# mohwald/gandtr

Hardware: AMD Instinct MI355X
Metric: images/sec generator@256^2 + descriptors/sec GeM-R101@1024^2, 1/2/4/8 MI355X (higher is better)
Workload: dtype f16c; 1 GPU; cyclegan ResnetGenerator 9-block (InstanceNorm) forward, synthetic 3x256x256, random-init weights; batch_per_gpu=64, global_batch=64, parallelism=dp1

## Files before the change

gandtr_amd/csrc/aux_kernels.hip:

```cpp
#include "gdt_common.h"
#include "aux_kernels.h"

namespace {

__device__ __forceinline__ void load8(const f16* p, float (&v)[8]) {
    const f16x8 t = *(const f16x8*)p;
#pragma unroll
    for (int e = 0; e < 8; ++e) v[e] = (float)t[e];
}
__device__ __forceinline__ void load8(const float* p, float (&v)[8]) {
    const float4 a = *(const float4*)p, b = *(const float4*)(p + 4);
    v[0] = a.x; v[1] = a.y; v[2] = a.z; v[3] = a.w; v[4] = b.x; v[5] = b.y; v[6] = b.z; v[7] = b.w;
}
__device__ __forceinline__ void store8(f16* p, const float (&v)[8]) {
    f16x8 t;
#pragma unroll
    for (int e = 0; e < 8; ++e) t[e] = (f16)v[e];
    *(f16x8*)p = t;
}
__device__ __forceinline__ void store8(float* p, const float (&v)[8]) {
    *(float4*)p = make_float4(v[0], v[1], v[2], v[3]);
    *(float4*)(p + 4) = make_float4(v[4], v[5], v[6], v[7]);
}

// ... 99 lines not shown
    var = var < 0.0 ? 0.0 : var;
    mean_rstd[(long)i * 2 + 0] = (float)m;
    mean_rstd[(long)i * 2 + 1] = (float)(1.0 / sqrt(var + (double)eps));
}

__global__ __launch_bounds__(1024) void in_finalize_tiles_kernel(const float* __restrict__ partial, float* __restrict__ mean_rstd,
                                                                 int tpi, int nphase, int N, int C, int HW, float eps) {
    constexpr int RL = 16;
    __shared__ double red[2][RL][64];
    const int n = blockIdx.y, c = blockIdx.x * 64 + (threadIdx.x & 63), lanegrp = threadIdx.x >> 6;
    double s = 0.0, q = 0.0;
    if (c < C) {
        const int nrec = nphase * tpi;
        auto rec = [&](int r, float& a, float& b) {
            if (r < nrec) {
                const int ph = r / tpi, t = r - ph * tpi;
                const long tile = (long)ph * N * tpi + (long)n * tpi + t;
                a = partial[(tile * 2 + 0) * C + c]; b = partial[(tile * 2 + 1) * C + c];
            } else { a = 0.f; b = 0.f; }
        };
        for (int r = lanegrp; r < nrec; r += 4 * RL) {
            float a0, b0, a1, b1, a2, b2, a3, b3;
            rec(r, a0, b0); rec(r + RL, a1, b1); rec(r + 2 * RL, a2, b2); rec(r + 3 * RL, a3, b3);
            s += (double)a0; q += (double)b0; s += (double)a1; q += (double)b1;
            s += (double)a2; q += (double)b2; s += (double)a3; q += (double)b3;
        }
    }
    red[0][lanegrp][threadIdx.x & 63] = s; red[1][lanegrp][threadIdx.x & 63] = q;
    __syncthreads();
    if (threadIdx.x < 64 && c < C) {
        s = 0.0; q = 0.0;
#pragma unroll
        for (int l = 0; l < RL; ++l) { s += red[0][l][threadIdx.x]; q += red[1][l][threadIdx.x]; }
        const double m = s / HW;
        double var = q / HW - m * m;
        var = var < 0.0 ? 0.0 : var;
        mean_rstd[((long)n * C + c) * 2 + 0] = (float)m;
        mean_rstd[((long)n * C + c) * 2 + 1] = (float)(1.0 / sqrt(var + (double)eps));
    }
}

template <typename T>
__global__ __launch_bounds__(256) void in_apply_kernel(const T* __restrict__ x, const float* __restrict__ mean_rstd,
                                                       const T* __restrict__ res, T* __restrict__ y,
                                                       long HW, int C, int relu, long total8) {
    const int c8n = C >> 3;
    for (long i = (long)blockIdx.x * 256 + threadIdx.x; i < total8; i += (long)gridDim.x * 256) {
        const int c8 = (int)(i % c8n);
        const long n = (i / c8n) / HW;
        const float* mr = mean_rstd + (n * C + c8 * 8) * 2;
        float v[8], r[8];
        load8(x + i * 8, v);
        if (res) load8(res + i * 8, r);
#pragma unroll
        for (int e = 0; e < 8; ++e) {
            float f = (v[e] - mr[2 * e]) * mr[2 * e + 1];
            if (relu) f = fmaxf(f, 0.f);
            if (res) f += r[e];
            v[e] = f;
        }
        store8(y + i * 8, v);
    }
}

template <typename T>
__global__ __launch_bounds__(256) void maxpool_kernel(const T* __restrict__ x, T* __restrict__ y, int N, int H, int W,
                                                      int C, int OH, int OW, int k, int s, int p) {
    const int c8n = C >> 3;
    const long total = (long)N * OH * OW * c8n;
    for (long i = (long)blockIdx.x * 256 + threadIdx.x; i < total; i += (long)gridDim.x * 256) {
        const int c8 = (int)(i % c8n);
// ... 542 lines not shown
```

gandtr_amd/csrc/conv3x3_halo_c16.hip:

```cpp
#include <cstdio>
#include <cstdlib>

#include <vector>

#include "gdt_common.h"

#ifndef GDT_C16_SCHED
#define GDT_C16_SCHED 1
#endif
#ifndef GDT_C16_RING
#define GDT_C16_RING 3
#endif
#ifndef GDT_C16_FULL_LINES
#define GDT_C16_FULL_LINES 1
#endif
#ifndef GDT_C16_BQ_SETS
#define GDT_C16_BQ_SETS 1
#endif
#ifndef GDT_C16_ABL
#define GDT_C16_ABL 0
#endif

namespace {

// ... 74 lines not shown
        int rx = ix < 0 ? -ix : (ix >= d.W ? 2 * d.W - 2 - ix : ix);
        ry = min(max(ry, 0), d.H - 1); rx = min(max(rx, 0), d.W - 1);
        const bool inb = ((unsigned)iy < (unsigned)d.H) & ((unsigned)ix < (unsigned)d.W);
        Pend p;
        p.goff = (((unsigned)((ta.n * d.H + ry) * d.W + rx) << (d.lc8 + 5)) + cbyte);
        p.ok = (h < HROWS) & (inb | refl);
        p.r0 = *(const float4*)((const char*)inf + p.goff); p.r1 = *(const float4*)((const char*)inf + p.goff + 16);
        if (RES) { p.s0 = *(const float4*)((const char*)resf + p.goff); p.s1 = *(const float4*)((const char*)resf + p.goff + 16); }
        return p;
    };
    Pend pendv[SDIST];
    auto load_piece_part = [&](const TileAt& ta, int chunk, int r, int part) {
        Pend& pend = pendv[r % SDIST];
        if (part == 0) {
            int lr = lrow;
            asm volatile("" : "+v"(lr));
            const int h = min(r * RPR + lr, HROWS_PAD - 1);
            const int hy = (h * 3641) >> 16, hx = h - hy * HW_;
            const int iy = ta.y0 - 1 + hy, ix = ta.x0 - 1 + hx;
            int ry = iy < 0 ? -iy : (iy >= d.H ? 2 * d.H - 2 - iy : iy);
            int rx = ix < 0 ? -ix : (ix >= d.W ? 2 * d.W - 2 - ix : ix);
            ry = min(max(ry, 0), d.H - 1); rx = min(max(rx, 0), d.W - 1);
            const bool inb = ((unsigned)iy < (unsigned)d.H) & ((unsigned)ix < (unsigned)d.W);
            pend.goff = (((unsigned)((ta.n * d.H + ry) * d.W + rx) << (d.lc8 + 5)) + (chunk * 8 + (lane & 7)) * 32);
            pend.ok = (h < HROWS) & (inb | refl);
            pend.r0 = *(const float4*)((const char*)inf + pend.goff);
        }
        if (part == 1) pend.r1 = *(const float4*)((const char*)inf + pend.goff + 16);
        if (RES && part == 2) pend.s0 = *(const float4*)((const char*)resf + pend.goff);
        if (RES && part == 3) pend.s1 = *(const float4*)((const char*)resf + pend.goff + 16);
    };
    float* nlds = (float*)(smem + 2 * STAGE_BYTES);
    auto stage_norm = [&](const TileAt& ta, int slot) {
        for (int i = tid; i < d.Cin / 2; i += NT) {
            const float4 v = *(const float4*)(d.in_norm + (long)ta.n * d.Cin * 2 + i * 4);
            *(float4*)(nlds + slot * 512 + i * 4) = make_float4(v.y, -v.x * v.y, v.w, -v.z * v.w);
        }
    };
    float4 nf[4];
    auto load_nf = [&](int slot, int chunk) {
        if (!NORM) return;
        const float4* np4 = (const float4*)(nlds + slot * 512 + (chunk * 8 + (lane & 7)) * 16);
#pragma unroll
        for (int k = 0; k < 4; ++k) nf[k] = np4[k];
    };
    auto store_piece = [&](int stage_off, int r, const Pend& p) {
        const int row = min(r * RPR + lrow, HROWS_PAD - 1);
        const int phy = (row * 3641) >> 16, phx = row - phy * HW_;
        float a[8] = {p.r0.x, p.r0.y, p.r0.z, p.r0.w, p.r1.x, p.r1.y, p.r1.z, p.r1.w};
        if (NORM) {
            const float lo = d.in_relu ? 0.f : -3.0e38f;
#pragma unroll
            for (int k = 0; k < 4; ++k) {
                const float4 v = nf[k];
                a[2 * k] = fmaxf(fmaf(a[2 * k], v.x, v.y), lo);
                a[2 * k + 1] = fmaxf(fmaf(a[2 * k + 1], v.z, v.w), lo);
            }
            if (RES) {
                a[0] += p.s0.x; a[1] += p.s0.y; a[2] += p.s0.z; a[3] += p.s0.w;
                a[4] += p.s1.x; a[5] += p.s1.y; a[6] += p.s1.z; a[7] += p.s1.w;
            }
        }
        if (WB) {
            *(float4*)((char*)wbf + p.goff) = make_float4(a[0], a[1], a[2], a[3]);
            *(float4*)((char*)wbf + p.goff + 16) = make_float4(a[4], a[5], a[6], a[7]);
        }
// ... 441 lines not shown
```

gandtr_amd/csrc/gdt_common.h:

```cpp
#pragma once
#include <hip/hip_runtime.h>
#include <hip/hip_fp16.h>
#include <stdint.h>
#include <mutex>
#include <string>

typedef _Float16 f16;
typedef f16 f16x8 __attribute__((ext_vector_type(8)));
typedef f16 f16x4 __attribute__((ext_vector_type(4)));
typedef f16 f16x2 __attribute__((ext_vector_type(2)));
typedef float f32x16 __attribute__((ext_vector_type(16)));
typedef float f32x4 __attribute__((ext_vector_type(4)));

void gdt_set_error(const std::string& msg);
#define GDT_OK 0
#define GDT_ERR_INVALID 1
#define GDT_ERR_HIP 2
#define GDT_ERR_WORKSPACE 3
#ifndef GDT_ERR_NOT_CONVERGED
#define GDT_ERR_NOT_CONVERGED 4
#endif

#define GDT_CHECK_HIP(expr)                                                                     \
    do {                                                                                        \
// ... 47 lines not shown
    float* stats;
    const f16* zeros;
    const float* in_norm;
    int in_relu;
    const f16* w_frag;
    const f16* in_res;
    f16* in_out;
    int N, H, W, Cin, lc8;
    int Cout, CoutPad, Kpad, nk;
    int OHg, OWg, OH, OW;
    int sy, sx, osy, ooy, osx, oox;
    int ntaps, TW, invTW, dy0, dys, dx0, dxs;
    int pad_reflect;
    int relu;
    int act;
    int M;
    int dbg;
    unsigned long long* stamp_out;
    int stats_tile_base;
    int pool2;
    const f16* w_frag2;
    const void* w_cfrag;
    const void* wmx_a; const void* wmx_b; const void* wmx_s;
    const void* w_c16;
    int pair_cout, ooy2, oox2;
    int x3_form;
    int in_f32;
    int stagger_us;
    int phase_cout;
    const f16* in2; int in2_cin, in2_h, in2_w, in2_stride;
    const f16* x_w_frag; const f16* x_bias; int x_cout;
    const f16* r_w_frag; const float* r_bias; f16* r_out;
    float group_factor;
};

constexpr int GDT_MAX_LEVELS = 4;

constexpr int GDT_C_HI_SCALE_OFF = 11;
__device__ __forceinline__ int gdt_c_pixel_exp(const float (&a)[8]) {
    const float m = fmaxf(fmaxf(fmaxf(fabsf(a[0]), fabsf(a[1])), fmaxf(fabsf(a[2]), fabsf(a[3]))),
                          fmaxf(fmaxf(fabsf(a[4]), fabsf(a[5])), fmaxf(fabsf(a[6]), fabsf(a[7]))));
    int b = __float_as_int(m);
    b = max(b, __builtin_amdgcn_mov_dpp(b, 0xB1, 0xF, 0xF, false));
    b = max(b, __builtin_amdgcn_mov_dpp(b, 0x4E, 0xF, 0xF, false));
    b = max(b, __builtin_amdgcn_mov_dpp(b, 0x141, 0xF, 0xF, false));
    return min(max((b >> 23) - 127, -14), 15);
}
__device__ __forceinline__ float gdt_exp2i(int e) { return __int_as_float((e + 127) << 23); }
struct MultiConv {
    int nlev;
    int prefix[GDT_MAX_LEVELS + 1];
    int vblocks[GDT_MAX_LEVELS];
    ConvLaunch lev[GDT_MAX_LEVELS];
};
static_assert(sizeof(MultiConv) <= 4096, "kernel arguments are limited to 4 KB");
__device__ __forceinline__ int gdt_multi_level(const int nlev, const int* prefix, const int b) {
    int l = 0;
#pragma unroll
    for (int k = 1; k < GDT_MAX_LEVELS; ++k) l += (k < nlev && b >= prefix[k]) ? 1 : 0;
    return l;
}
inline int gdt_multi_partition(int* prefix, const int* vb, int L, int slots) {
    long total = 0;
    for (int l = 0; l < L; ++l) total += vb[l];
    prefix[0] = 0;
    for (int l = 0; l < L; ++l) {
        int g = vb[l];
        if (total > slots) {
            g = (int)((long)slots * vb[l] / total) / 8 * 8;
            if (g < 8) g = 8;
            if (g > vb[l]) g = vb[l];
        }
        prefix[l + 1] = prefix[l] + g;
    }
    return prefix[L];
}

__device__ __forceinline__ bool gdt_tile_of_block(int b, int ntm, int ntn, int& tile_m, int& tile_n) {
    const int mchunk = (ntm + 7) >> 3;
    const int xcd = b & 7, j = b >> 3;
    tile_n = j % ntn;
// ... 69 lines not shown
```

gandtr_amd/csrc/net.hip:

```cpp
#include <algorithm>
#include <cmath>
#include <cstdlib>
#include <cstring>
#include <memory>
#include <vector>

#include "../../include/gandtr_hip.h"
#include "aux_kernels.h"
#include "gdt_common.h"

static thread_local std::string g_last_error;
void gdt_set_error(const std::string& msg) { g_last_error = msg; }

namespace {

constexpr size_t ALIGN = 256;
inline size_t align_up(size_t v) { return (v + ALIGN - 1) / ALIGN * ALIGN; }
inline int next_pow2(int v) { int p = 8; while (p < v) p <<= 1; return p; }
inline int ilog2(int v) { int l = 0; while ((1 << l) < v) ++l; return l; }

enum OpKind { OP_INPUT, OP_CONV, OP_INORM, OP_MAXPOOL, OP_GEM, OP_OUT_NCHW, OP_HED, OP_RCF, OP_POOL_HEAD };

struct PackedPhase {
    size_t w_off = 0;
// ... 108 lines not shown
    int last_joined = 0, last_level_launches = 0;

    size_t blob_append(const void* data, size_t bytes) {
        const size_t off = align_up(host_blob.size());
        host_blob.resize(off + bytes);
        if (data) memcpy(host_blob.data() + off, data, bytes);
        else memset(host_blob.data() + off, 0, bytes);
        return off;
    }
    int new_tensor(int C, int Creal) { tensors.push_back(Tensor{C, Creal}); return (int)tensors.size() - 1; }
};

namespace {

struct Step {
    int op; size_t aux_off[8]; bool fused_stats; int tiles_per_image;
    int norm_into;
    int norm_from;
    bool wb;
    bool ctf;
    bool aug;
    bool s2;
    bool ctp;
    int pool_into;
    bool skip;
    bool bneck;
    int bneck_ds;
    int bneck_a;
    bool xexp;
    int xchain;
    bool kcat;
    bool direct;
    int stats_sets;
};
struct Plan { std::vector<Step> steps; size_t peak = 0; };

int pool_out_dim(const Op& o, int in) {
    const int span = in + 2 * o.p - o.k + (o.ceil ? o.s - 1 : 0);
    if (span < 0) return 0;
    int out = span / o.s + 1;
    if (o.ceil && (out - 1) * o.s >= in + o.p) --out;
    return out;
}

int conv_out_dim(const Op& o, int in, int k) {
    const gdt_conv_desc& c = o.cd;
    if (c.transposed) return in * 2;
    const int span = in + 2 * c.pad - (o.dil * (k - 1) + 1);
    return span < 0 ? 0 : span / c.stride + 1;
}

void conv_geometry(const gdt_net* net, const Op& o, const PackedPhase& ph, int n, const Tensor& ti, ConvLaunch& d) {
    d.N = n; d.H = ti.H; d.W = ti.W; d.Cin = o.cin_pad; d.lc8 = ilog2(o.cin_pad / 8);
    d.Cout = o.cd.cout; d.CoutPad = o.cout_pad;
    d.OH = conv_out_dim(o, ti.H, o.cd.kh); d.OW = conv_out_dim(o, ti.W, o.cd.kw);
    d.pad_reflect = o.cd.pad_reflect; d.relu = o.cd.relu; d.act = o.cd.act;
    d.Kpad = ph.Kpad; d.nk = ph.Kpad / (net->precision ? 32 : 64);
    d.ntaps = ph.ntaps; d.TW = ph.TW; d.invTW = (65536 + ph.TW - 1) / ph.TW;
    d.dy0 = ph.dy0; d.dys = ph.dys; d.dx0 = ph.dx0; d.dxs = ph.dxs;
    if (o.cd.transposed) {
        d.OHg = ti.H; d.OWg = ti.W; d.sy = d.sx = 1; d.osy = d.osx = 2; d.ooy = ph.ooy; d.oox = ph.oox;
    } else {
        d.OHg = d.OH; d.OWg = d.OW; d.sy = d.sx = o.cd.stride; d.osy = d.osx = 1; d.ooy = d.oox = 0;
    }
    d.M = n * d.OHg * d.OWg;
}
// ... 216 lines not shown
            d.w_frag = (const f16*)net; d.out = (f16*)net;
            d.stats = conv_fuses_stats(ok, T[ok.in]) ? (float*)net : nullptr;
            ConvLaunch dn = d; dn.in_norm = (const float*)net; dn.in_res = oj.res >= 0 ? (const f16*)net : nullptr;
            const bool ok_fold = consumers[oj.out] == 1 && (gdt_conv_halo_ct_eligible(dn) || (oj.res < 0 && gdt_conv_igemm_rb_eligible(dn)));
            if (ok_fold) { plan.steps[j].norm_into = k; plan.steps[k].norm_from = j; plan.steps[j].wb = false; }
            continue;
        }
        conv_geometry(net, ok, ok.phases[0], N, T[ok.in], d);
        if (ok.rowsplit) { d.Cout = ok.rs_cout8; d.out_f32 = nullptr; }
        d.w_lo = net->precision ? (const f16*)net : nullptr;
        d.w_frag = ok.phases[0].has_frag ? (const f16*)net : nullptr;
        d.out = (ok.cd.out_f32_nchw || ok.rowsplit) ? nullptr : (f16*)net;
        d.stats = conv_fuses_stats(ok, T[ok.in]) ? (float*)net : nullptr;
        d.out_f32 = (ok.cd.out_f32_nchw && !ok.rowsplit) ? (float*)net : nullptr;
        const bool fold = net->precision ? (((x3_fold >= 2 || (!wb && oj.res < 0)) && gdt_conv_halo_x3_eligible(d)) ||
                                            (x3_fold >= 2 && !wb && oj.res < 0 && !ok.rowsplit && !ok.cd.out_f32_nchw && gdt_conv_x3_norm_eligible(d)))
                                         : (gdt_conv_halo_eligible(d) || (!wb && (gdt_conv_igemm_norm_eligible(d) || irb_norm_ok(d))));
        if (fold) { plan.steps[j].norm_into = k; plan.steps[k].norm_from = j; plan.steps[j].wb = wb; }
        static const bool plan_dbg = getenv("GDT_PLAN_DEBUG") != nullptr;
        if (plan_dbg) fprintf(stderr, "[plan] inorm %d -> conv %d: Cin %d s%d k%d rowsplit %d fold %d\n", j, k, d.Cin, ok.cd.stride, ok.cd.kh, (int)ok.rowsplit, (int)fold);
    }

    for (int i = 0; i < nops; ++i) {
        const Op& o = ops[i];
        if (o.kind != OP_CONV || plan.steps[i].ctf || o.cd.transposed || o.rowsplit || o.cd.out_f32_nchw || net->precision) continue;
        if (!conv_fuses_stats(o, T[o.in])) continue;
        ConvLaunch d{};
        conv_geometry(net, o, o.phases[0], N, T[o.in], d);
        d.w_frag = o.phases[0].has_frag ? (const f16*)net : nullptr; d.out = (f16*)net; d.stats = (float*)net;
        d.in_norm = plan.steps[i].norm_from >= 0 ? (const float*)net : nullptr;
        if (plan.steps[i].norm_from >= 0 && plan.steps[plan.steps[i].norm_from].wb) continue;
        if (!gdt_conv_stem_eligible(d) && !gdt_conv_halo_rb_eligible(d) && !gdt_conv_halo_eligible(d) && gdt_conv_igemm_rb_eligible(d))
            plan.steps[i].stats_sets = gdt_conv_igemm_rb_stats_sets(d);
    }

    for (int j = 0; j < nops; ++j) {
        const Op& oj = ops[j];
        if (oj.kind != OP_MAXPOOL || oj.k != 2 || oj.s != 2 || oj.p != 0 || net->precision || consumers[oj.in] != 1) continue;
        if (oj.ceil && ((T[oj.in].H & 1) || (T[oj.in].W & 1))) continue;
        int i = -1;
        for (int k = 0; k < j; ++k) if (ops[k].kind == OP_CONV && ops[k].out == oj.in) i = k;
        if (i < 0 || ops[i].cd.transposed || ops[i].cd.out_f32_nchw || ops[i].res >= 0 || ops[i].dil != 1) continue;
        ConvLaunch d{};
        conv_geometry(net, ops[i], ops[i].phases[0], N, T[ops[i].in], d);
        d.w_frag = ops[i].phases[0].has_frag ? (const f16*)net : nullptr; d.out = (f16*)net;
        d.in_norm = plan.steps[i].norm_from >= 0 ? (const float*)net : nullptr;
        d.stats = conv_fuses_stats(ops[i], T[ops[i].in]) ? (float*)net : nullptr;
        if (plan.steps[i].norm_from >= 0 && plan.steps[plan.steps[i].norm_from].wb) continue;
        if (gdt_conv_pool2_eligible(d)) { plan.steps[i].pool_into = j; plan.steps[j].skip = true; }
    }

    for (int i = 0; i + 2 < nops && !net->precision; ++i) {
        const Op &a = ops[i], &b = ops[i + 1], &c = ops[i + 2];
        if (a.kind != OP_CONV || b.kind != OP_CONV || c.kind != OP_CONV) continue;
        auto plain = [&](const Op& o) { return o.dil == 1 && !o.cd.transposed && !o.cd.out_f32_nchw && !o.rowsplit && o.stats_for < 0 && o.cd.stride == 1 && o.phases.size() == 1 && o.phases[0].has_frag && o.has_bias; };
        if (!plain(a) || !plain(b) || !plain(c)) continue;
        if (a.cd.kh != 1 || a.cd.kw != 1 || a.cd.pad != 0 || !a.cd.relu || a.res >= 0) continue;
        if (b.cd.kh != 3 || b.cd.kw != 3 || b.cd.pad != 1 || b.cd.pad_reflect || !b.cd.relu || b.res >= 0 || b.in != a.out) continue;
        if (c.cd.kh != 1 || c.cd.kw != 1 || c.cd.pad != 0 || !c.cd.relu || c.in != b.out || c.res != a.in) continue;
        if (consumers[a.out] != 1 || consumers[b.out] != 1) continue;
        if (plan.steps[i].norm_from >= 0 || plan.steps[i + 1].norm_from >= 0 || plan.steps[i + 2].norm_from >= 0) continue;
        if (plan.steps[i].pool_into >= 0 || plan.steps[i + 1].pool_into >= 0 || plan.steps[i + 2].pool_into >= 0) continue;
        const int C = a.cd.cin, mid = a.cd.cout;
        if (a.cin_pad != C || a.cout_pad != mid || b.cd.cin != mid || b.cd.cout != mid || b.cout_pad != mid || c.cd.cin != mid || c.cd.cout != C || c.cout_pad != C) continue;
        if (!gdt_bneck_eligible(C, C, mid, N, T[a.in].H, T[a.in].W)) continue;
        plan.steps[i].bneck = true; plan.steps[i + 1].skip = true; plan.steps[i + 2].skip = true;
// ... 134 lines not shown
                        t2.off = arena.alloc(t2.bytes);
                    }
                    break;
                }
                if (st.pool_into >= 0) {
                    Tensor& t = T[ops[st.pool_into].out];
                    t.bytes = (size_t)N * t.H * t.W * t.C * net->esize();
                    t.off = arena.alloc(t.bytes);
                } else if (o.out >= 0) alloc_out();
                if (o.rowsplit) {
                    const size_t b = (size_t)N * oh * ti.W * o.rs_cout8 * net->esize();
                    st.aux_off[1] = arena.alloc(b);
                    arena.release(st.aux_off[1], b);
                }
                if (conv_fuses_stats(o, ti)) {
                    const int hwg = o.cd.transposed ? ti.H * ti.W : oh * conv_out_dim(o, ti.W, o.cd.kw);
                    const size_t tiles = (size_t)st.stats_sets * N * (hwg / 128);
                    st.fused_stats = true; st.tiles_per_image = hwg / 128;
                    slab_bytes[i] = tiles * 2 * o.cd.cout * sizeof(float);
                    st.aux_off[0] = arena.alloc(slab_bytes[i]);
                    slab_off[i] = st.aux_off[0];
                }
                break;
            }
            case OP_INORM: {
                const Tensor& ti = T[o.in];
                const size_t mr_bytes = (size_t)N * ti.C * 2 * sizeof(float);
                if (st.norm_into < 0 || st.wb) alloc_out();
                st.aux_off[1] = arena.alloc(mr_bytes);
                if (o.stats_from >= 0 && slab_bytes[o.stats_from]) {
                    st.fused_stats = true;
                    st.tiles_per_image = plan.steps[o.stats_from].tiles_per_image;
                    st.aux_off[0] = slab_off[o.stats_from];
                    arena.release(slab_off[o.stats_from], slab_bytes[o.stats_from]);
                } else {
                    const int chunks = gdt_in_stats_chunks(ti.H * ti.W);
                    st.aux_off[0] = arena.alloc((size_t)N * chunks * 2 * ti.C * sizeof(float));
                    arena.release(st.aux_off[0], (size_t)N * chunks * 2 * ti.C * sizeof(float));
                }
                if (st.norm_into >= 0) deferred[st.norm_into].push_back({st.aux_off[1], mr_bytes});
                else arena.release(st.aux_off[1], mr_bytes);
                break;
            }
            case OP_MAXPOOL: if (!st.skip) alloc_out(); break;
            case OP_GEM: {
                const Tensor& ti = T[o.in];
                st.aux_off[0] = arena.alloc((size_t)N * ti.C * sizeof(float));
                arena.release(st.aux_off[0], (size_t)N * ti.C * sizeof(float));
                break;
            }
            case OP_POOL_HEAD: {
                const Tensor& ti = T[o.in];
                std::vector<GdtPoolBox> boxes;
                const int rc = gdt_pool_grid(ti.H, ti.W, o.pool_aggregate ? o.pool_levels : 0, boxes);
                if (rc != GDT_OK) return rc;
                GDT_REQUIRE((int)boxes.size() <= GDT_POOL_MAX_REGIONS, "pool head: more than 64 regions per image for this map size");
                const size_t b = gdt_pool_head_scratch_floats(N, (int)boxes.size(), ti.C) * sizeof(float);
                st.aux_off[0] = arena.alloc(b);
                arena.release(st.aux_off[0], b);
                break;
            }
            case OP_OUT_NCHW: break;
            case OP_HED: {
                size_t sz[5];
                for (int k = 0; k < 5; ++k) {
                    const Tensor& tf = T[o.feats[k]];
                    sz[k] = (size_t)N * tf.H * tf.W * sizeof(float);
                    st.aux_off[k] = arena.alloc(sz[k]);
// ... 809 lines not shown
        for (int t : o.feats) { const Tensor& tf = net->tensors[t]; f += 2.0 * n * tf.H * tf.W * tf.Creal; }
        return f;
    }
    return 0.0;
}

static double op_bytes(const gdt_net* net, const Op& o, int n) {
    if (o.kind != OP_CONV) return 0.0;
    const double es = (double)net->esize();
    const Tensor& ti = net->tensors[o.in];
    const double oh = conv_out_dim(o, ti.H, o.cd.kh), ow = conv_out_dim(o, ti.W, o.cd.kw);
    const double out_b = (double)n * oh * ow * o.cd.cout * (o.cd.out_f32_nchw ? 4.0 : es);
    double in_px = (double)n * ti.H * ti.W;
    if (!o.cd.transposed && o.cd.kh == 1 && o.cd.kw == 1 && o.cd.stride > 1) in_px = (double)n * oh * ow;
    double b = in_px * ti.C * es + out_b;
    if (o.res >= 0) b += out_b;
    b += (double)o.cd.cin * o.cd.cout * o.cd.kh * o.cd.kw * sizeof(f16);
    return b;
}

int gdt_net_plan_summary(gdt_net* net, int n, int rh, int rw, int resize, int* counts, int n_counts) {
    GDT_REQUIRE(net && counts && n_counts >= 10 && n >= 1 && rh >= 1 && rw >= 1, "plan summary arguments");
    if (!net->finalized && !net->precision) build_kcat_weights(net);
    Plan plan;
    int rc = make_plan(net, n, rh, rw, plan, resize == 0);
    if (rc != GDT_OK) return rc;
    for (int k = 0; k < n_counts; ++k) counts[k] = 0;
    for (size_t i = 0; i < plan.steps.size(); ++i) {
        const Step& st = plan.steps[i];
        const Op& o = net->ops[i];
        if (o.kind == OP_CONV && !st.skip) ++counts[0];
        if (o.kind == OP_CONV) { counts[1] += st.bneck; counts[2] += st.xexp; counts[3] += st.xchain >= 0; counts[4] += st.kcat; counts[8] += st.ctf; counts[9] += st.s2; }
        if (o.kind == OP_INORM) counts[5] += st.norm_into >= 0;
        if (o.kind == OP_MAXPOOL) counts[6] += st.skip;
        if (o.kind == OP_POOL_HEAD && n_counts >= 14) {
            counts[12] += 1 + (o.pool_aggregate ? 2 + (o.has_rw ? 2 : 0) + (o.pool_aggregate == 2 ? 1 : 0) : 1) + (o.has_fw ? 2 : 0);
            counts[13] += 1;
        }
        if (o.kind == OP_INPUT) counts[7] += st.direct;
        if (o.kind == OP_CONV && o.dil != 1 && n_counts >= 12) {
            ++counts[10];
            ConvLaunch d{};
            conv_geometry(net, o, o.phases[0], n, net->tensors[o.in], d);
            d.w_frag = o.phases[0].has_frag ? (const f16*)net : nullptr; d.w_lo = net->precision ? (const f16*)net : nullptr; d.out = (f16*)net;
            if (o.phases[0].has_mx) d.w_cfrag = d.wmx_a = d.wmx_b = d.wmx_s = net;
            counts[11] += st.skip || st.bneck || st.xexp || st.pool_into >= 0 || st.s2 || st.aug || st.direct || gdt_conv_halo_eligible(d) ||
                          gdt_conv_halo_rb_eligible(d) || gdt_conv_halo_x3_eligible(d) || gdt_conv_halo_x3_taps_eligible(d) || gdt_conv_halo_c_eligible(d) ||
                          gdt_conv_stem_eligible(d) || gdt_conv_stem_c_eligible(d) || gdt_conv_1x1_rb_eligible(d);
        }
    }
    return GDT_OK;
}

int gdt_net_flops(gdt_net* net, int n, int rh, int rw, double* flops) {
    GDT_REQUIRE(net && flops, "net");
    Plan plan;
    int rc = make_plan(net, n, rh, rw, plan);
    if (rc != GDT_OK) return rc;
    double f = 0.0;
    for (const Op& o : net->ops) f += op_flops(net, o, n, rh, rw);
    *flops = f;
    return GDT_OK;
}

int gdt_net_set_profiling(gdt_net* net, int enable) {
    GDT_REQUIRE(net && net->finalized, "net must be finalized");
// ... 147 lines not shown
                            const double yb = (double)n * T[a2.in].H * T[a2.in].W * T[a2.in].C * (double)net->esize();
                            net->last_flops[stp.op] += net->last_flops[stp.xchain]; net->last_flops[stp.xchain] = 0.0;
                            net->last_bytes[stp.op] += net->last_bytes[stp.xchain] - yb; net->last_bytes[stp.xchain] = 0.0;
                        }
                    }
                    break;
                }
                if (stp.kcat) {
                    const Op& ds = net->ops[o.kcat_ds];
                    ConvLaunch d{};
                    conv_geometry(net, o, o.phases[0], n, ti, d);
                    d.in = tptr(o.in); d.out = tptr(o.out); d.zeros = zeros;
                    d.w_frag = (const f16*)(net->dev_blob + o.kcat_frag_off);
                    d.bias = (const float*)(net->dev_blob + o.kcat_bias_off);
                    d.Kpad = o.cin_pad + ds.cin_pad; d.nk = d.Kpad / 64;
                    d.in2 = tptr(ds.in); d.in2_cin = ds.cin_pad; d.in2_h = T[ds.in].H; d.in2_w = T[ds.in].W; d.in2_stride = ds.cd.stride;
                    if (defer) { defer->kind = DEFER_CONV; defer->kcat = true; defer->d = d; }
                    else rc = gdt_launch_conv_1x1_rb(d, st);
                    if (net->profiling && book) {
                        net->last_variant[stp.op] = 946128;
                        net->last_flops[stp.op] += net->last_flops[o.kcat_ds]; net->last_flops[o.kcat_ds] = 0.0;
                        const double proj = (double)n * T[o.out].H * T[o.out].W * T[o.out].C * (double)net->esize();
                        net->last_bytes[stp.op] += net->last_bytes[o.kcat_ds] - 2.0 * proj; net->last_bytes[o.kcat_ds] = 0.0;
                    }
                    break;
                }
                ConvLaunch d{};
                d.in = tptr(o.in);
                if (stp.norm_from >= 0) {
                    const Op& nj = net->ops[stp.norm_from];
                    d.in = tptr(nj.in);
                    d.in_norm = (const float*)(ws + plan.steps[stp.norm_from].aux_off[1]);
                    d.in_relu = nj.relu;
                    if (nj.res >= 0) d.in_res = tptr(nj.res);
                    if (plan.steps[stp.norm_from].wb) d.in_out = tptr(nj.out);
                    if (net->profiling) {
                        const double tb = (double)n * T[nj.in].H * T[nj.in].W * T[nj.in].C * (double)net->esize();
                        net->last_bytes[stp.op] += tb * ((nj.res >= 0 ? 1.0 : 0.0) + (plan.steps[stp.norm_from].wb ? 1.0 : 0.0));
                    }
                }
                d.res = o.res >= 0 ? tptr(o.res) : nullptr;
                d.zeros = zeros;
                d.stats = stp.fused_stats ? (float*)(ws + stp.aux_off[0]) : nullptr;
                if (stp.ctf) {
                    ctf_geometry(net, o, n, ti, d);
                    d.bias = o.has_bias ? (const float*)(net->dev_blob + o.ctf_bias_off) : nullptr;
                    d.out = tptr(o.out); d.out_f32 = nullptr;
                    d.w = nullptr; d.w_lo = nullptr; d.w_frag = o.ctf.has_frag ? (const f16*)(net->dev_blob + o.ctf.w_frag_off) : nullptr;
                    d.stats_tile_base = 0;
                    int variant = 960256;
                    if (net->precision == 2) {
                        d.w_cfrag = net->dev_blob + o.ctf.wc_off; d.wmx_a = net->dev_blob + o.ctf.wmx_a_off; d.wmx_b = net->dev_blob + o.ctf.wmx_b_off; d.wmx_s = net->dev_blob + o.ctf.wmx_s_off;
                        variant = 980256;
                        rc = gdt_launch_conv_halo_c_ct(d, st);
                    } else
                    rc = gdt_conv_halo_ct_eligible(d) ? gdt_launch_conv_halo_ct(d, st) : gdt_launch_conv_igemm_rb(d, st, &variant);
                    if (net->profiling) net->last_variant[stp.op] = variant;
                    break;
                }
                if (stp.s2) {
                    s2_geometry(net, o, n, ti, d);
                    d.bias = o.has_bias ? (const float*)(net->dev_blob + o.s2_bias_off) : nullptr;
                    d.out = tptr(o.out); d.out_f32 = nullptr; d.w = nullptr; d.w_lo = nullptr; d.w_frag = nullptr;
                    d.stats_tile_base = 0;
                    if (net->precision == 1) {
                        d.w = (const f16*)(net->dev_blob + o.s2.w_off); d.w_lo = (const f16*)(net->dev_blob + o.s2.w_lo_off); d.x3_form = 2;
// ... 29 lines not shown
                for (const PackedPhase& ph : o.phases) {
                    conv_geometry(net, o, ph, n, ti, d);
                    d.bias = o.has_bias ? (const float*)(net->dev_blob + o.bias_off) : nullptr;
                    if (o.rowsplit) { d.out = (f16*)(ws + stp.aux_off[1]); d.out_f32 = nullptr; d.Cout = o.rs_cout8; d.bias = nullptr; }
                    else if (o.cd.out_f32_nchw) { d.out = nullptr; d.out_f32 = (float*)outputs[o.slot]; }
                    else if (stp.pool_into >= 0) { d.out = tptr(net->ops[stp.pool_into].out); d.out_f32 = nullptr; d.pool2 = 1; }
                    else { d.out = tptr(o.out); d.out_f32 = nullptr; }
                    d.w = (const f16*)(net->dev_blob + ph.w_off);
                    d.w_lo = f32 ? (const f16*)(net->dev_blob + ph.w_lo_off) : nullptr;
                    d.w_frag = ph.has_frag ? (const f16*)(net->dev_blob + ph.w_frag_off) : nullptr;
                    if (ph.has_mx) {
                        d.w_cfrag = net->dev_blob + ph.wc_off; d.wmx_a = net->dev_blob + ph.wmx_a_off; d.wmx_b = net->dev_blob + ph.wmx_b_off; d.wmx_s = net->dev_blob + ph.wmx_s_off;
                    }
                    if (ph.has_mx16) {
                        d.w_c16 = net->dev_blob + ph.w16_off;
                    }
                    d.stats_tile_base = phase_idx * (d.M / 128);
                    ++phase_idx;
                    int variant = 0;
                    if (o.rowsplit) {
                        ConvLaunch h = d;
                        h.out = nullptr; h.out_f32 = (float*)outputs[o.slot]; h.Cout = o.cd.cout; h.act = o.cd.act; h.in_f32 = f32;
                        h.w_frag2 = (net->precision == 1 && ph.has_frag) ? (const f16*)(net->dev_blob + ph.w_frag2_off) : nullptr;
                        h.bias = o.has_bias ? (const float*)(net->dev_blob + o.rs_bias_off) : nullptr;
                        if (gdt_conv_head7_eligible(h)) {
                            rc = gdt_launch_conv_head7(h, st);
                            if (net->profiling) net->last_variant[stp.op] = 920007;
                            fused_head = true;
                            break;
                        }
                    }
                    if (stp.aug) { d.w_frag2 = (const f16*)(net->dev_blob + ph.w_frag2_off); variant = 955000 + ph.ntaps; rc = gdt_launch_conv_stem_c(d, st); }
                    else if (net->precision == 2 && gdt_conv_halo_c16_eligible(d)) { variant = 971256; rc = gdt_launch_conv_halo_c16(d, st); }
                    else if (net->precision == 2 && gdt_conv_halo_c_eligible(d)) { variant = 970000 + gdt_conv_halo_c_columns(d); rc = gdt_launch_conv_halo_c(d, st); }
                    else if (defer && !f32 && o.phases.size() == 1 && !o.rowsplit && !o.cd.out_f32_nchw) { defer->kind = DEFER_CONV; defer->kcat = false; defer->d = d; }
                    else rc = f32 ? gdt_launch_conv_x3(d, st, &variant) : gdt_launch_conv(d, st, &variant);
                    if (net->profiling) net->last_variant[stp.op] = variant;
                    if (rc != GDT_OK) break;
                }
                if (o.rowsplit && !fused_head && rc == GDT_OK)
                    rc = gdt_k_rowsplit_combine(d.out, f32, o.has_bias ? (const float*)(net->dev_blob + o.rs_bias_off) : nullptr,
                                                (float*)outputs[o.slot], n, d.OH, ti.W, o.rs_cout8, o.cd.cout, o.cd.kw, o.cd.pad,
                                                o.cd.pad_reflect, o.cd.act, st);
                break;
            }
            case OP_INORM: {
                const Tensor& ti = T[o.in];
                if (stp.norm_into >= 0)
                    rc = gdt_k_instance_norm_stats(tptr(o.in), f32, stp.fused_stats, (float*)(ws + stp.aux_off[0]), stp.tiles_per_image,
                                                   stp.fused_stats ? plan.steps[o.stats_from].stats_sets : 1,
                                                   (float*)(ws + stp.aux_off[1]), n, ti.H * ti.W, ti.C, o.eps, st);
                else if (stp.fused_stats)
                    rc = gdt_k_instance_norm_fused(tptr(o.in), o.res >= 0 ? tptr(o.res) : nullptr, tptr(o.out), f32,
                                                   (const float*)(ws + stp.aux_off[0]), stp.tiles_per_image,
                                                   plan.steps[o.stats_from].stats_sets, (float*)(ws + stp.aux_off[1]), n,
                                                   ti.H * ti.W, ti.C, o.eps, o.relu, st);
                else
                    rc = gdt_k_instance_norm(tptr(o.in), o.res >= 0 ? tptr(o.res) : nullptr, tptr(o.out), f32, (float*)(ws + stp.aux_off[0]),
                                             (float*)(ws + stp.aux_off[1]), n, ti.H * ti.W, ti.C, o.eps, o.relu, st);
                break;
            }
            case OP_MAXPOOL: {
                if (stp.skip) break;
                const Tensor& ti = T[o.in]; const Tensor& to = T[o.out];
                rc = gdt_k_maxpool(tptr(o.in), tptr(o.out), f32, n, ti.H, ti.W, ti.C, to.H, to.W, o.k, o.s, o.p, st);
                break;
            }
            case OP_GEM: {
                const Tensor& ti = T[o.in];
                rc = gdt_k_gem_l2n(tptr(o.in), f32, (float*)(ws + stp.aux_off[0]), (float*)outputs[o.slot], n, ti.H * ti.W, ti.C, o.gem_p,
                                   o.eps_gem, o.eps_l2, st);
                break;
            }
            case OP_POOL_HEAD: {
                const Tensor& ti = T[o.in];
                std::vector<GdtPoolBox> boxes;
                GdtPoolRegions g{};
                rc = gdt_pool_grid(ti.H, ti.W, o.pool_aggregate ? o.pool_levels : 0, boxes);
                if (rc == GDT_OK) rc = gdt_pool_regions_of(boxes, g);
                if (rc != GDT_OK) break;
// ... 222 lines not shown
```

gandtr_amd/engine.py:

```python
import collections
import ctypes
import math
import os

import numpy as np
import torch

from . import _hip
from ._hip import ConvDesc


def _f32(t):
    if t is None:
        return None
    if isinstance(t, torch.Tensor):
        t = t.detach().to("cpu", torch.float32).contiguous().numpy()
    return np.ascontiguousarray(t, dtype=np.float32)


def _ptr(a):
    return None if a is None else a.ctypes.data_as(ctypes.c_void_p)


_SIDE_STREAMS = {}
# ... 112 lines not shown
    def hed_head(self, feats, score_w, score_b, fusion_w, fusion_b, sigmoid=True):
        ws = [_f32(w).reshape(-1) for w in score_w]
        wp = (ctypes.c_void_p * 5)(*[w.ctypes.data for w in ws])
        out = ctypes.c_int()
        _hip.check(self.lib.gdt_net_hed_head(self.handle, (ctypes.c_int * 5)(*feats), wp,
                                             (ctypes.c_float * 5)(*[float(b) for b in score_b]),
                                             (ctypes.c_float * 5)(*[float(w) for w in fusion_w]), float(fusion_b),
                                             int(sigmoid), ctypes.byref(out)))
        return out.value

    def rcf_head(self, feats, stage_of, side_w, stage_b, fuse_w, fuse_b, sigmoid=True):
        if len(feats) != 13 or len(stage_of) != 13 or len(side_w) != 13 or len(stage_b) != 5 or len(fuse_w) != 5:
            raise ValueError("the RCF head takes 13 features (and stages / side vectors) and 5 stage biases / fusion weights")
        ws = [_f32(w).reshape(-1) for w in side_w]
        wp = (ctypes.c_void_p * 13)(*[w.ctypes.data for w in ws])
        out = ctypes.c_int()
        _hip.check(self.lib.gdt_net_rcf_head(self.handle, (ctypes.c_int * 13)(*feats), (ctypes.c_int * 13)(*stage_of), wp,
                                             (ctypes.c_float * 5)(*[float(b) for b in stage_b]),
                                             (ctypes.c_float * 5)(*[float(w) for w in fuse_w]), float(fuse_b), int(sigmoid), ctypes.byref(out)))
        return out.value

    def finalize(self):
        with torch.cuda.device(self.device):
            _hip.check(self.lib.gdt_net_finalize(self.handle))
        self._finalized = True
        return self

    @staticmethod
    def resized_size(h, w, scale):
        if scale is None:
            return h, w
        return int(math.floor(float(h * scale))), int(math.floor(float(w * scale)))

    _PLAN_KNOBS = ("GDT_CONV_XEXP", "GDT_XEXP_CHAIN", "GDT_CONV_BNECK", "GDT_CONV_HALO_X3", "GDT_CONV_HALO_X3_FORMS", "GDT_X3_NORM_FOLD")

    def _geometry(self, n, rh, rw):
        key = (n, rh, rw, getattr(self, "_group_factor", 1.0)) + tuple(os.environ.get(k) for k in self._PLAN_KNOBS)
        cache = self.__dict__.setdefault("_geo_cache", {})
        hit = cache.get(key)
        if hit is None:
            b = ctypes.c_size_t()
            _hip.check(self.lib.gdt_net_workspace_bytes(self.handle, n, rh, rw, ctypes.byref(b)))
            shapes = []
            dims, ndim = (ctypes.c_int * 4)(), ctypes.c_int()
            for slot in range(self.lib.gdt_net_num_outputs(self.handle)):
                _hip.check(self.lib.gdt_net_output_shape(self.handle, slot, n, rh, rw, dims, ctypes.byref(ndim)))
                shapes.append(tuple(dims[i] for i in range(ndim.value)))
            if len(cache) > 256:
                cache.clear()
            hit = (b.value, shapes)
            if self._finalized:
                cache[key] = hit
        return hit

    def output_shapes(self, n, rh, rw):
        return list(self._geometry(n, rh, rw)[1])

    PLAN_KEYS = ("conv_launches", "bottlenecks_fused", "conv3x3_expand", "chained_reduce", "shortcuts_folded", "norms_folded", "pools_fused", "direct_stem",
                 "transposed_fused", "stride2_shift", "dilated_convs", "dilated_special_forms")

    def plan_summary(self, n, rh, rw, resize=False):
        c = (ctypes.c_int * 12)()
        _hip.check(self.lib.gdt_net_plan_summary(self.handle, n, rh, rw, int(bool(resize)), c, 12))
        return dict(zip(self.PLAN_KEYS, list(c)))

    def head_launches(self, n, rh, rw):
        c = (ctypes.c_int * 14)()
# ... 477 lines not shown
```

Before: 6019 images/s.

## Merge instance-norm statistics finalize into consuming c16 halo conv prologue

```diff
diff --git a/gandtr_amd/csrc/aux_kernels.hip b/gandtr_amd/csrc/aux_kernels.hip
--- a/gandtr_amd/csrc/aux_kernels.hip
+++ b/gandtr_amd/csrc/aux_kernels.hip
@@ -155,11 +155,10 @@
         s = 0.0; q = 0.0;
 #pragma unroll
         for (int l = 0; l < RL; ++l) { s += red[0][l][threadIdx.x]; q += red[1][l][threadIdx.x]; }
-        const double m = s / HW;
-        double var = q / HW - m * m;
-        var = var < 0.0 ? 0.0 : var;
-        mean_rstd[((long)n * C + c) * 2 + 0] = (float)m;
-        mean_rstd[((long)n * C + c) * 2 + 1] = (float)(1.0 / sqrt(var + (double)eps));
+        float mean, rstd;
+        gdt_in_mean_rstd(s, q, HW, eps, mean, rstd);
+        mean_rstd[((long)n * C + c) * 2 + 0] = mean;
+        mean_rstd[((long)n * C + c) * 2 + 1] = rstd;
     }
 }
 
diff --git a/gandtr_amd/csrc/conv3x3_halo_c16.hip b/gandtr_amd/csrc/conv3x3_halo_c16.hip
--- a/gandtr_amd/csrc/conv3x3_halo_c16.hip
+++ b/gandtr_amd/csrc/conv3x3_halo_c16.hip
@@ -130,6 +130,18 @@
     };
     float* nlds = (float*)(smem + 2 * STAGE_BYTES);
     auto stage_norm = [&](const TileAt& ta, int slot) {
+        if (d.in_stats) {
+            int cin = d.Cin;
+            asm volatile("" : "+s"(cin));
+            for (int c = tid; c < d.Cin; c += NT) {
+                double s, q;
+                gdt_in_merge_records(d.in_stats, d.in_stats_tpi, d.in_stats_sets, d.N, cin, ta.n, c, s, q);
+                float mean, rstd;
+                gdt_in_mean_rstd(s, q, d.in_stats_hw, d.in_stats_eps, mean, rstd);
+                *(float2*)(nlds + slot * 512 + c * 2) = make_float2(rstd, -mean * rstd);
+            }
+            return;
+        }
         for (int i = tid; i < d.Cin / 2; i += NT) {
             const float4 v = *(const float4*)(d.in_norm + (long)ta.n * d.Cin * 2 + i * 4);
             *(float4*)(nlds + slot * 512 + i * 4) = make_float4(v.y, -v.x * v.y, v.w, -v.z * v.w);
diff --git a/gandtr_amd/csrc/gdt_common.h b/gandtr_amd/csrc/gdt_common.h
--- a/gandtr_amd/csrc/gdt_common.h
+++ b/gandtr_amd/csrc/gdt_common.h
@@ -103,6 +103,7 @@
     const f16* x_w_frag; const f16* x_bias; int x_cout;
     const f16* r_w_frag; const float* r_bias; f16* r_out;
     float group_factor;
+    const float* in_stats; int in_stats_tpi, in_stats_sets, in_stats_hw; float in_stats_eps;
 };
 
 constexpr int GDT_MAX_LEVELS = 4;
@@ -118,6 +119,45 @@
     return min(max((b >> 23) - 127, -14), 15);
 }
 __device__ __forceinline__ float gdt_exp2i(int e) { return __int_as_float((e + 127) << 23); }
+__device__ __forceinline__ void gdt_in_mean_rstd(double s, double q, int HW, float eps, float& mean, float& rstd) {
+    const double m = s / HW;
+    double var = q / HW - m * m;
+    var = var < 0.0 ? 0.0 : var;
+    mean = (float)m;
+    rstd = (float)(1.0 / sqrt(var + (double)eps));
+}
+__device__ __forceinline__ void gdt_in_merge_records(const float* __restrict__ partial, int tpi, int nphase, int N, int C, int n, int c, double& s, double& q) {
+    const int nrec = nphase * tpi;
+    auto at = [&](int r) -> const float* {
+        const int ph = r / tpi, t = r - ph * tpi;
+        return partial + (((long)ph * N * tpi + (long)n * tpi + t) * 2) * C + c;
+    };
+    s = 0.0; q = 0.0;
+    if (nphase == 1 && nrec == 32) {
+        const float* pa = partial + ((long)n * tpi * 2) * C + c;
+        const float* pb = pa + C;
+        float a[32], b[32];
+#pragma unroll
+        for (int r = 0; r < 32; ++r) {
+            asm volatile("" : "+v"(pa), "+v"(pb));
+            a[r] = *pa; b[r] = *pb;
+            pa += 2l * C; pb += 2l * C;
+        }
+#pragma unroll
+        for (int l = 0; l < 16; ++l) {
+            double sl = 0.0, ql = 0.0;
+            sl += (double)a[l]; ql += (double)b[l];
+            sl += (double)a[l + 16]; ql += (double)b[l + 16];
+            s += sl; q += ql;
+        }
+        return;
+    }
+    for (int l = 0; l < 16; ++l) {
+        double sl = 0.0, ql = 0.0;
+        for (int r = l; r < nrec; r += 16) { const float* p = at(r); sl += (double)p[0]; ql += (double)p[C]; }
+        s += sl; q += ql;
+    }
+}
 struct MultiConv {
     int nlev;
     int prefix[GDT_MAX_LEVELS + 1];
diff --git a/gandtr_amd/csrc/net.hip b/gandtr_amd/csrc/net.hip
--- a/gandtr_amd/csrc/net.hip
+++ b/gandtr_amd/csrc/net.hip
@@ -164,6 +164,7 @@
     bool kcat;
     bool direct;
     int stats_sets;
+    bool merge;
 };
 struct Plan { std::vector<Step> steps; size_t peak = 0; };
 
@@ -446,6 +447,26 @@
         if (plan.steps[i].norm_from >= 0 && plan.steps[plan.steps[i].norm_from].wb) continue;
         if (!gdt_conv_stem_eligible(d) && !gdt_conv_halo_rb_eligible(d) && !gdt_conv_halo_eligible(d) && gdt_conv_igemm_rb_eligible(d))
             plan.steps[i].stats_sets = gdt_conv_igemm_rb_stats_sets(d);
+    }
+
+    {
+        const char* merge_env = getenv("GDT_NORM_MERGE");
+        const bool merge_on = !merge_env || atoi(merge_env) != 0;
+        for (int j = 0; j < nops && merge_on && net->precision == 2; ++j) {
+            const Op& oj = ops[j];
+            const int k = plan.steps[j].norm_into;
+            if (oj.kind != OP_INORM || k < 0 || oj.stats_from < 0) continue;
+            const Op& ok = ops[k];
+            if (plan.steps[k].ctf || plan.steps[k].s2 || plan.steps[k].ctp || plan.steps[k].aug || ok.cd.transposed || ok.rowsplit || ok.cd.out_f32_nchw ||
+                ok.phases.size() != 1 || !ok.phases[0].has_mx || !ok.phases[0].has_mx16 || T[oj.in].C != ok.cin_pad) continue;
+            ConvLaunch d{};
+            conv_geometry(net, ok, ok.phases[0], N, T[ok.in], d);
+            d.w = (const f16*)net; d.w_cfrag = d.wmx_a = d.wmx_b = d.wmx_s = net; d.w_c16 = net; d.out = (f16*)net;
+            d.res = ok.res >= 0 ? (const f16*)net : nullptr;
+            d.stats = conv_fuses_stats(ok, T[ok.in]) ? (float*)net : nullptr;
+            d.in_norm = (const float*)net; d.in_res = oj.res >= 0 ? (const f16*)net : nullptr; d.in_out = plan.steps[j].wb ? (f16*)net : nullptr;
+            plan.steps[j].merge = gdt_conv_halo_c16_eligible(d);
+        }
     }
 
     for (int j = 0; j < nops; ++j) {
@@ -646,8 +667,10 @@
                     st.fused_stats = true;
                     st.tiles_per_image = plan.steps[o.stats_from].tiles_per_image;
                     st.aux_off[0] = slab_off[o.stats_from];
-                    arena.release(slab_off[o.stats_from], slab_bytes[o.stats_from]);
+                    if (st.merge) deferred[st.norm_into].push_back({slab_off[o.stats_from], slab_bytes[o.stats_from]});
+                    else arena.release(slab_off[o.stats_from], slab_bytes[o.stats_from]);
                 } else {
+                    st.merge = false;
                     const int chunks = gdt_in_stats_chunks(ti.H * ti.W);
                     st.aux_off[0] = arena.alloc((size_t)N * chunks * 2 * ti.C * sizeof(float));
                     arena.release(st.aux_off[0], (size_t)N * chunks * 2 * ti.C * sizeof(float));
@@ -1523,6 +1546,7 @@
         if (o.kind == OP_CONV && !st.skip) ++counts[0];
         if (o.kind == OP_CONV) { counts[1] += st.bneck; counts[2] += st.xexp; counts[3] += st.xchain >= 0; counts[4] += st.kcat; counts[8] += st.ctf; counts[9] += st.s2; }
         if (o.kind == OP_INORM) counts[5] += st.norm_into >= 0;
+        if (o.kind == OP_INORM && n_counts >= 16) { counts[14] += st.merge; counts[15] += st.fused_stats && !st.merge; }
         if (o.kind == OP_MAXPOOL) counts[6] += st.skip;
         if (o.kind == OP_POOL_HEAD && n_counts >= 14) {
             counts[12] += 1 + (o.pool_aggregate ? 2 + (o.has_rw ? 2 : 0) + (o.pool_aggregate == 2 ? 1 : 0) : 1) + (o.has_fw ? 2 : 0);
@@ -1736,6 +1760,12 @@
                     d.in = tptr(nj.in);
                     d.in_norm = (const float*)(ws + plan.steps[stp.norm_from].aux_off[1]);
                     d.in_relu = nj.relu;
+                    if (plan.steps[stp.norm_from].merge) {
+                        const Step& sn = plan.steps[stp.norm_from];
+                        d.in_stats = (const float*)(ws + sn.aux_off[0]);
+                        d.in_stats_tpi = sn.tiles_per_image; d.in_stats_sets = plan.steps[nj.stats_from].stats_sets;
+                        d.in_stats_hw = T[nj.in].H * T[nj.in].W; d.in_stats_eps = nj.eps;
+                    }
                     if (nj.res >= 0) d.in_res = tptr(nj.res);
                     if (plan.steps[stp.norm_from].wb) d.in_out = tptr(nj.out);
                     if (net->profiling) {
@@ -1831,6 +1861,7 @@
                     }
                     if (stp.aug) { d.w_frag2 = (const f16*)(net->dev_blob + ph.w_frag2_off); variant = 955000 + ph.ntaps; rc = gdt_launch_conv_stem_c(d, st); }
                     else if (net->precision == 2 && gdt_conv_halo_c16_eligible(d)) { variant = 971256; rc = gdt_launch_conv_halo_c16(d, st); }
+                    else if (d.in_stats) { gdt_set_error("planner: a norm without a finalize launch feeds a conv that does not merge statistics records"); rc = GDT_ERR_INVALID; }
                     else if (net->precision == 2 && gdt_conv_halo_c_eligible(d)) { variant = 970000 + gdt_conv_halo_c_columns(d); rc = gdt_launch_conv_halo_c(d, st); }
                     else if (defer && !f32 && o.phases.size() == 1 && !o.rowsplit && !o.cd.out_f32_nchw) { defer->kind = DEFER_CONV; defer->kcat = false; defer->d = d; }
                     else rc = f32 ? gdt_launch_conv_x3(d, st, &variant) : gdt_launch_conv(d, st, &variant);
@@ -1845,6 +1876,7 @@
             }
             case OP_INORM: {
                 const Tensor& ti = T[o.in];
+                if (stp.merge) break;
                 if (stp.norm_into >= 0)
                     rc = gdt_k_instance_norm_stats(tptr(o.in), f32, stp.fused_stats, (float*)(ws + stp.aux_off[0]), stp.tiles_per_image,
                                                    stp.fused_stats ? plan.steps[o.stats_from].stats_sets : 1,
diff --git a/gandtr_amd/engine.py b/gandtr_amd/engine.py
--- a/gandtr_amd/engine.py
+++ b/gandtr_amd/engine.py
@@ -168,7 +168,7 @@
             return h, w
         return int(math.floor(float(h * scale))), int(math.floor(float(w * scale)))
 
-    _PLAN_KNOBS = ("GDT_CONV_XEXP", "GDT_XEXP_CHAIN", "GDT_CONV_BNECK", "GDT_CONV_HALO_X3", "GDT_CONV_HALO_X3_FORMS", "GDT_X3_NORM_FOLD")
+    _PLAN_KNOBS = ("GDT_CONV_XEXP", "GDT_XEXP_CHAIN", "GDT_CONV_BNECK", "GDT_CONV_HALO_X3", "GDT_CONV_HALO_X3_FORMS", "GDT_X3_NORM_FOLD", "GDT_NORM_MERGE")
 
     def _geometry(self, n, rh, rw):
         key = (n, rh, rw, getattr(self, "_group_factor", 1.0)) + tuple(os.environ.get(k) for k in self._PLAN_KNOBS)
```

Result: no change. 5985 images/s (-0.6%).
